# NVIDIAGameWorks/RayTracingDenoiser

Measured on AMD Instinct MI355X. Metric: Mpixels/s REBLUR_DIFFUSE_SPECULAR @1440p, higher is better.
Workload: dtype f32; 1 GPU; REBLUR_DIFFUSE_SPECULAR 2560x1440, default settings, analytic scene + 1rpp noise, moving camera; parallelism=1 GPU, storage=reference pool formats (fp16 history, R10G10B10A2 normals)

## Files before the change

raytracingdenoiser_amd/csrc/hip/kernels_reblur_ta.hip:

```cpp
#include "passes.h"
#include <climits>
#include <cstdio>
#include "reblur_device.h"

namespace nrdhip {

constexpr int TILE_X = 32;
constexpr int TILE_Y = 8;
static_assert(TILE_X == 32 && TILE_Y == 8, "planes.h LoadBlockTileBytes: a workgroup covers two 16x16 tiles of one tile row");
constexpr int BORDER = 1;
constexpr int BUF_X = TILE_X + 2 * BORDER;
constexpr int BUF_Y = TILE_Y + 2 * BORDER;
constexpr int BUF_STRIDE = BUF_X + 1;

#ifndef NRD_TA_WIN_H
#define NRD_TA_WIN_W 64
#define NRD_TA_WIN_H 16
#endif
#ifndef NRD_TA_SKY_FLAG_STORE
#define NRD_TA_SKY_FLAG_STORE 1
#endif
constexpr int WIN_W = NRD_TA_WIN_W;
constexpr int WIN_H = NRD_TA_WIN_H;

// ... 12 lines not shown
template <typename T>
NRD_D void WindowHistoryTexels(const HistoryFilter&, const uint2*, int, int, int, T&) {}
NRD_D void WindowFastTexels(const HistoryFilter& h, const uint32_t* win, int wx0, int wy0, const Plane& dims, int shift, BilinearTexelsR16F& t) {
    const int x0 = ClampI(h.ox, 0, dims.w - 1) - wx0, x1 = ClampI(h.ox + 1, 0, dims.w - 1) - wx0;
    const int y0 = (ClampI(h.oy, 0, dims.h - 1) - wy0) * WIN_W, y1 = (ClampI(h.oy + 1, 0, dims.h - 1) - wy0) * WIN_W;
    const uint32_t f00 = InBounds(dims, h.ox, h.oy) ? (win[y0 + x0] >> shift) & 0xFFFFu : 0u, f10 = InBounds(dims, h.ox + 1, h.oy) ? (win[y0 + x1] >> shift) & 0xFFFFu : 0u;
    const uint32_t f01 = InBounds(dims, h.ox, h.oy + 1) ? (win[y1 + x0] >> shift) & 0xFFFFu : 0u, f11 = InBounds(dims, h.ox + 1, h.oy + 1) ? (win[y1 + x1] >> shift) & 0xFFFFu : 0u;
    t.r0 = f00 | (f10 << 16);
    t.r1 = f01 | (f11 << 16);
    t.loaded = true;
}
template <typename T>
NRD_D void WindowFastTexels(const HistoryFilter&, const uint32_t*, int, int, const Plane&, int, T&) {}


template <bool DIFF, bool SPEC, bool PERF, int KIND, bool SH, int MODE>
__device__ __forceinline__ void ReblurTemporalAccumulationTile(const ReblurCB& cArg, TaPlanes P, const RowRange& rr, const int tileX, const int blockY) {
    typedef ReblurSignal<KIND> Sig;
    constexpr bool OCC = KIND == SIGNAL_OCCLUSION;
    typedef typename Sig::type S;
    __shared__ float4 s_Normal_Roughness[BUF_Y * BUF_STRIDE];
    __shared__ ReblurCB s_Constants;

    {
        const Plane size = P.viewZ, rgba16 = DIFF ? P.historyDiff : P.historySpec, r16 = DIFF ? P.historyDiffFast : P.historySpecFast;
        ShareSize(P.decodedNR, size), ShareSize(P.mv, size), ShareSize(P.prevViewZ, size), ShareSize(P.prevNormalRoughness, size), ShareSize(P.prevInternalData, size);
        ShareSize(P.inDiff, size), ShareSize(P.inSpec, size), ShareSize(P.inSpecHitDistForTracking, size), ShareSize(P.outData1, size), ShareSize(P.outData2, size);
        if (OCC) {
            const Plane sig = DIFF ? P.outDiff : P.outSpec;
            ShareSize(P.historyDiff, size), ShareSize(P.historySpec, size), ShareLayout(P.outDiff, sig), ShareLayout(P.outSpec, sig);
        } else {
            ShareLayout(P.historyDiff, rgba16), ShareLayout(P.historySpec, rgba16), ShareLayout(P.outDiff, rgba16), ShareLayout(P.outSpec, rgba16);
        }
        ShareLayout(P.historyDiffFast, r16), ShareLayout(P.historySpecFast, r16), ShareLayout(P.prevSpecHitDistForTracking, r16), ShareLayout(P.outDiffFast, r16), ShareLayout(P.outSpecFast, r16),
            ShareLayout(P.outSpecHitDistForTracking, r16);
    }
    __shared__ float s_HitDistForTracking[BUF_Y * BUF_STRIDE];
    constexpr int WIN_TEXELS = MODE == 1 ? WIN_W * WIN_H : 1;
    __shared__ float s_WinZ[WIN_TEXELS];
    __shared__ NrRaw s_WinN[WIN_TEXELS];
    __shared__ uint32_t s_WinId[WIN_TEXELS];
    __shared__ uint32_t s_WinFast[WIN_TEXELS];
    __shared__ uint2 s_WinDiff[WIN_TEXELS], s_WinSpec[WIN_TEXELS];
    __shared__ int s_WinBox[4][4];

    const int tx = threadIdx.x % TILE_X, ty = threadIdx.x / TILE_X;
    uint8_t* const tileFlag = (MODE == 1 && tileX < P.tileFlags.w && blockY < P.tileFlags.h) ? P.tileFlags.ptr + (uint32_t)blockY * P.tileFlags.pitch + (uint32_t)tileX : nullptr;
    const int px = tileX * TILE_X + tx, py = blockY * TILE_Y + ty;
    const int rw = cArg.gRectSizeMinusOne.x, rh = cArg.gRectSizeMinusOne.y;

    float preViewZ = 0.0f, preMaterialID = 0.0f;
    float4 preMv = F4(0.0f), preNormalAndRoughness = F4(0.0f);
    const uint32_t tileBytes = LoadBlockTileBytes(P.tiles, tileX, blockY);
    const bool preSky = TileByteIsSky(tileBytes, tx >> 4);
    {
        if (!TileBytesHaveGeometry<2>(tileBytes)) {
            if (NRD_TA_SKY_FLAG_STORE && MODE == 1 && threadIdx.x == 0 && tileFlag)
                *tileFlag = 0;
            return;
        }

        if (MODE == 1) {
            const int qx = min(px, rw), qy = min(max(py, 0), rh);
            preViewZ = LoadR32F(P.viewZ, qx, qy);
            preMv = LoadRGBA16F(P.mv, qx, qy);
            preNormalAndRoughness = LoadDecodedNormalRoughness(P.decodedNR, qx, qy, preMaterialID);
        }
        const int baseX = tileX * TILE_X - BORDER, baseY = blockY * TILE_Y - BORDER;
        for (int i = threadIdx.x; i < BUF_X * BUF_Y; i += TILE_X * TILE_Y) {
            int lx = i % BUF_X, ly = i / BUF_X;
            int gx = ClampI(baseX + lx, 0, rw), gy = ClampI(baseY + ly, 0, rh);
            float unusedMaterialID, texelViewZ;
            s_Normal_Roughness[ly * BUF_STRIDE + lx] = LoadDecodedNormalRoughness(P.decodedNR, gx, gy, unusedMaterialID, texelViewZ);
            if (SPEC) {
                const int shift = (OCC && cArg.gSpecCheckerboard != 2) ? 1 : 0;
                float hitDist = (OCC || cArg.gSpecPrepassBlurRadius == 0.0f) ? ExtractHitDist(Sig::Load(P.inSpec, gx >> shift, gy)) : LoadR16F(P.inSpecHitDistForTracking, gx, gy);
                if (shift) {
                    const int sx = min((gx & ~1) | (int)((cArg.gSpecCheckerboard ^ (uint32_t)gy ^ cArg.gFrameIndex) & 1u), rw);
                    LoadDecodedNormalRoughness(P.decodedNR, sx, gy, unusedMaterialID, texelViewZ);
                }
                if ((OCC || cArg.gSpecPrepassBlurRadius == 0.0f) && texelViewZ > cArg.gDenoisingRange)
                    hitDist = 0.0f;
                s_HitDistForTracking[ly * BUF_STRIDE + lx] = hitDist == 0.0f ? NRD_INF : hitDist;
            }
        }
        const uint32_t __attribute__((address_space(4)))* kernarg = (const uint32_t __attribute__((address_space(4)))*)__builtin_amdgcn_kernarg_segment_ptr();
        if (threadIdx.x < sizeof(ReblurCB) / 4)
            ((uint32_t*)&s_Constants)[threadIdx.x] = kernarg[threadIdx.x];
    }
    __syncthreads();
    const ReblurCB& c = s_Constants;
#define NRD_CONSTANTS_PHASE() asm volatile("" ::: "memory")

    const int lpx = MODE == 1 ? min(px, rw) : px, lpy = MODE == 1 ? min(py, rh) : py;
    bool active = !(px > rw || py > rh || py < rr.rowBegin || py >= rr.rowEnd);
    if (MODE != 1 && !active)
        return;
    if (MODE != 1) {
        if (preSky)
            return;
        preViewZ = LoadR32F(P.viewZ, lpx, lpy);
    }
    active = active && !preSky;
    const float viewZ = UnpackViewZ(c, preViewZ);
    active = active && !(viewZ > c.gDenoisingRange);
    if (MODE != 1 && !active)
        return;

    const float2 rectSize = ToF2(c.gRectSize), rectSizeInv = ToF2(c.gRectSizeInv), rectSizePrev = ToF2(c.gRectSizePrev);
    const float3 cameraDelta = ToF3(c.gCameraDelta);
    const float4 frustum = ToF4(c.gFrustum), frustumPrev = ToF4(c.gFrustumPrev), hitDistParams = ToF4(c.gHitDistParams);

    float2 pixelUv = F2(float(px) + 0.5f, float(py) + 0.5f) * rectSizeInv;
    float3 Xv = ReconstructViewPosition(pixelUv, frustum, viewZ, NRD_ORTHO_MODE(c));
    float3 X = RotateVector(c.gViewToWorld, Xv);

    float3 Navg = F3(0.0f);
    float hitDistForTracking = NRD_INF, roughnessM1 = 0.0f, roughnessM2 = 0.0f;
#pragma unroll
    for (int j = 0; j <= 2; j++) {
#pragma unroll
        for (int i = 0; i <= 2; i++) {
            int o = (ty + j) * BUF_STRIDE + tx + i;
            float4 nr = s_Normal_Roughness[o];
            if (i < 2 && j < 2)
                Navg = Navg + Xyz(nr);
            if (SPEC) {
                hitDistForTracking = Min(hitDistForTracking, s_HitDistForTracking[o]);
                float roughnessSq = nr.w * nr.w;
                roughnessM1 += roughnessSq;
                roughnessM2 += roughnessSq * roughnessSq;
            }
        }
    }
    Navg = Navg * 0.25f;

    if (MODE != 1)
        preNormalAndRoughness = LoadDecodedNormalRoughness(P.decodedNR, lpx, lpy, preMaterialID);
    float materialID = preMaterialID;
    float4 normalAndRoughness = preNormalAndRoughness;
    float3 N = Xyz(normalAndRoughness);
    float roughness = normalAndRoughness.w;

    float roughnessModified = 0.0f, roughnessSigma = 0.0f, hitDistNormalization = 0.0f;
    RngHash rng;
    if (SPEC) {
        roughnessModified = GetModifiedRoughnessFromNormalVariance(roughness, Navg);
        roughnessM1 = roughnessM1 * (1.0f / 9.0f);
        roughnessM2 = roughnessM2 * (1.0f / 9.0f);
        roughnessSigma = Sqrt(Abs(roughnessM2 - roughnessM1 * roughnessM1));

        rng.Initialize((uint32_t)px, (uint32_t)py, c.gFrameIndex);

        hitDistForTracking = hitDistForTracking == NRD_INF ? 0.0f : hitDistForTracking;
        hitDistNormalization = GetHitDistanceNormalization(viewZ, hitDistParams, roughness);
        hitDistForTracking *= (OCC || c.gSpecPrepassBlurRadius == 0.0f) ? hitDistNormalization : 1.0f;
        if (active)
            StoreR16F(P.outSpecHitDistForTracking, px, py, hitDistForTracking);
    }

    NRD_CONSTANTS_PHASE();
    float4 mvRaw = MODE == 1 ? preMv : LoadRGBA16F(P.mv, lpx, lpy);
    float3 mv = F3(mvRaw.x, mvRaw.y, mvRaw.z) * F3(c.gMvScale.x, c.gMvScale.y, c.gMvScale.z);
    float3 Xprev = X;
    float2 smbPixelUv = pixelUv + F2(mv.x, mv.y);
    if (c.gMvScale.w == 0.0f) {
        if (c.gMvScale.z == 0.0f)
            mv.z = AffineTransform(c.gWorldToViewPrev, X).z - viewZ;
        float viewZprev = viewZ + mv.z;
        float3 Xvprevlocal = ReconstructViewPosition(smbPixelUv, frustumPrev, viewZprev, NRD_ORTHO_MODE(c));
        Xprev = RotateVectorInverse(c.gWorldToViewPrev, Xvprevlocal) + cameraDelta;
    } else {
        Xprev = Xprev + mv;
        smbPixelUv = GetScreenUv(c.gWorldToClipPrev, Xprev);
    }

    TrackHistoryReach(P.historyReach, active ? HistoryReachRows(smbPixelUv.y, rectSizePrev.y, py) : 0.0f);

    float2 catromOrigin = GetCatmullRomOrigin(smbPixelUv, rectSizePrev);
    const int cx = (int)catromOrigin.x, cy = (int)catromOrigin.y;
    Bilinear smbBilinearFilter = GetBilinearFilter(smbPixelUv, rectSizePrev);
    const int bx = (int)smbBilinearFilter.origin.x, by = (int)smbBilinearFilter.origin.y;
    const float2 smbSamplePos = Sat(smbPixelUv) * rectSizePrev;
    HistoryFilter smbFilter = MakeHistoryGeometry(smbSamplePos, DIFF ? P.historyDiff : P.historySpec);
    typename Sig::HistoryTexels smbDiffTexels, smbSpecTexels;
    typename Sig::FastTexels smbDiffFastTexels, smbSpecFastTexels;
    S diff = Sig::Zero(), spec = Sig::Zero();
    float4 smbViewZ0, smbViewZ1, smbViewZ2, smbViewZ3;
    uint32_t id0[4], id1[4], id2[4], id3[4];
    NrRaw n00, n10, n01, n11;
    int wx0 = 0, wy0 = 0;
    if (MODE == 1) {
        const int W1 = P.prevViewZ.w - 1, H1 = P.prevViewZ.h - 1;
        int loX = INT_MAX, loY = INT_MAX, hiX = INT_MIN, hiY = INT_MIN;
        if (active) {
            loX = min(min(ClampI(cx, 0, W1), ClampI(bx, 0, W1)), min(smbFilter.x[0], ClampI(smbFilter.ox, 0, W1)));
            hiX = max(max(ClampI(cx + 3, 0, W1), ClampI(bx + 1, 0, W1)), max(smbFilter.x[3], ClampI(smbFilter.ox + 1, 0, W1)));
            loY = min(min(ClampI(cy, 0, H1), ClampI(by, 0, H1)), min(smbFilter.y[0], ClampI(smbFilter.oy, 0, H1)));
            hiY = max(max(ClampI(cy + 3, 0, H1), ClampI(by + 1, 0, H1)), max(smbFilter.y[3], ClampI(smbFilter.oy + 1, 0, H1)));
        }
#pragma unroll
        for (int m = 32; m >= 1; m >>= 1) {
            loX = min(loX, __shfl_xor(loX, m)), loY = min(loY, __shfl_xor(loY, m));
            hiX = max(hiX, __shfl_xor(hiX, m)), hiY = max(hiY, __shfl_xor(hiY, m));
        }
        const int lane = threadIdx.x & 63, wave = threadIdx.x >> 6;
        if (lane == 0)
            s_WinBox[wave][0] = loX, s_WinBox[wave][1] = loY, s_WinBox[wave][2] = hiX, s_WinBox[wave][3] = hiY;
        __syncthreads();
        loX = min(min(s_WinBox[0][0], s_WinBox[1][0]), min(s_WinBox[2][0], s_WinBox[3][0]));
        loY = min(min(s_WinBox[0][1], s_WinBox[1][1]), min(s_WinBox[2][1], s_WinBox[3][1]));
        hiX = max(max(s_WinBox[0][2], s_WinBox[1][2]), max(s_WinBox[2][2], s_WinBox[3][2]));
        hiY = max(max(s_WinBox[0][3], s_WinBox[1][3]), max(s_WinBox[2][3], s_WinBox[3][3]));
        const bool empty = hiX < loX;
        const int bw = hiX - loX + 1, bh = hiY - loY + 1;
        if (empty || bw > P.winMaxW || bh > P.winMaxH) {
            if (threadIdx.x == 0 && tileFlag)
                *tileFlag = empty ? 0 : 1;
            return;
        }
        if (threadIdx.x == 0 && tileFlag)
            *tileFlag = 0;
        wx0 = loX, wy0 = loY;
        if (lane < bw)
            for (int r = wave; r < bh; r += 4) {
                const int x = wx0 + lane, y = wy0 + r, o = r * WIN_W + lane;
                s_WinZ[o] = LoadR32F(P.prevViewZ, x, y);
                s_WinN[o] = LoadNrRaw(P.prevNormalRoughness, x, y);
                s_WinId[o] = LoadR16U(P.prevInternalData, x, y);
                s_WinFast[o] = (DIFF ? LoadR16U(P.historyDiffFast, x, y) : 0u) | (SPEC ? LoadR16U(P.historySpecFast, x, y) << 16 : 0u);
                if (DIFF)
                    s_WinDiff[o] = *TexelPtr<const uint2>(P.historyDiff, x, y);
                if (SPEC)
                    s_WinSpec[o] = *TexelPtr<const uint2>(P.historySpec, x, y);
            }
        __syncthreads();
        if (!active)
            return;
        int xo[4], yo[4];
#pragma unroll
        for (int i = 0; i < 4; i++)
            xo[i] = ClampI(cx + i, 0, W1) - wx0, yo[i] = (ClampI(cy + i, 0, H1) - wy0) * WIN_W;
#define WIN_Z(i, j) s_WinZ[yo[j] + xo[i]]
#define WIN_ID(i, j) s_WinId[yo[j] + xo[i]]
        smbViewZ0 = F4(WIN_Z(0, 0), WIN_Z(1, 0), WIN_Z(0, 1), WIN_Z(1, 1)), smbViewZ1 = F4(WIN_Z(2, 0), WIN_Z(3, 0), WIN_Z(2, 1), WIN_Z(3, 1));
        smbViewZ2 = F4(WIN_Z(0, 2), WIN_Z(1, 2), WIN_Z(0, 3), WIN_Z(1, 3)), smbViewZ3 = F4(WIN_Z(2, 2), WIN_Z(3, 2), WIN_Z(2, 3), WIN_Z(3, 3));
        id0[0] = WIN_ID(0, 0), id0[1] = WIN_ID(1, 0), id0[2] = WIN_ID(0, 1), id0[3] = WIN_ID(1, 1);
        id1[0] = WIN_ID(2, 0), id1[1] = WIN_ID(3, 0), id1[2] = WIN_ID(2, 1), id1[3] = WIN_ID(3, 1);
        id2[0] = WIN_ID(0, 2), id2[1] = WIN_ID(1, 2), id2[2] = WIN_ID(0, 3), id2[3] = WIN_ID(1, 3);
        id3[0] = WIN_ID(2, 2), id3[1] = WIN_ID(3, 2), id3[2] = WIN_ID(2, 3), id3[3] = WIN_ID(3, 3);
#undef WIN_Z
#undef WIN_ID
        const int nx0 = ClampI(bx, 0, W1) - wx0, nx1 = ClampI(bx + 1, 0, W1) - wx0, ny0 = (ClampI(by, 0, H1) - wy0) * WIN_W, ny1 = (ClampI(by + 1, 0, H1) - wy0) * WIN_W;
        n00 = InBounds(P.prevNormalRoughness, bx, by) ? s_WinN[ny0 + nx0] : NrRawZero();
        n10 = InBounds(P.prevNormalRoughness, bx + 1, by) ? s_WinN[ny0 + nx1] : NrRawZero();
        n01 = InBounds(P.prevNormalRoughness, bx, by + 1) ? s_WinN[ny1 + nx0] : NrRawZero();
        n11 = InBounds(P.prevNormalRoughness, bx + 1, by + 1) ? s_WinN[ny1 + nx1] : NrRawZero();
    } else {
        const bool footprintInterior = FootprintIsInterior(P.prevViewZ, cx, cy, 4, 4);
        const int fx4 = max(0, min(cx, P.prevViewZ.w - 4));
        const int fy0 = ClampI(cy, 0, P.prevViewZ.h - 1), fy1 = ClampI(cy + 1, 0, P.prevViewZ.h - 1), fy2 = ClampI(cy + 2, 0, P.prevViewZ.h - 1), fy3 = ClampI(cy + 3, 0, P.prevViewZ.h - 1);
        const float4 zr0 = LoadRowR32Fx4(P.prevViewZ, fx4, fy0), zr1 = LoadRowR32Fx4(P.prevViewZ, fx4, fy1), zr2 = LoadRowR32Fx4(P.prevViewZ, fx4, fy2), zr3 = LoadRowR32Fx4(P.prevViewZ, fx4, fy3);
        const uint2 ir0 = LoadRowR16x4Raw(P.prevInternalData, fx4, fy0), ir1 = LoadRowR16x4Raw(P.prevInternalData, fx4, fy1), ir2 = LoadRowR16x4Raw(P.prevInternalData, fx4, fy2), ir3 = LoadRowR16x4Raw(P.prevInternalData, fx4, fy3);
        const bool normalsInterior = FootprintIsInterior(P.prevNormalRoughness, bx, by, 2, 2);
        {
            const int nx = max(0, min(bx, P.prevNormalRoughness.w - 2));
            LoadRowNrRawx2(P.prevNormalRoughness, nx, ClampI(by, 0, P.prevNormalRoughness.h - 1), n00, n10);
            LoadRowNrRawx2(P.prevNormalRoughness, nx, ClampI(by + 1, 0, P.prevNormalRoughness.h - 1), n01, n11);
        }
        if (DIFF) {
            Sig::PrefetchHistory(smbFilter, P.historyDiff, smbDiffTexels, !PERF && KIND != SIGNAL_DIRECTIONAL_OCCLUSION);
            Sig::PrefetchFast(smbFilter, P.historyDiffFast, smbDiffFastTexels);
// ... 138 lines not shown
    int cbX0 = 0, cbX1 = 0;
    float2 wc = F2(0.0f, 0.0f);
    if (OCC && (c.gDiffCheckerboard != 2 || c.gSpecCheckerboard != 2)) {
        const int x0 = px > 0 ? px - 1 : 0, x1 = px < c.gRectSizeMinusOne.x ? px + 1 : c.gRectSizeMinusOne.x;
        const float viewZ0 = UnpackViewZ(c, LoadR32F(P.viewZ, x0, py)), viewZ1 = UnpackViewZ(c, LoadR32F(P.viewZ, x1, py));
        const float thr = GetDisocclusionThreshold(NRD_DISOCCLUSION_THRESHOLD, frustumSize, NoV);
        wc = F2(thr >= Abs(viewZ0 - viewZ) ? 1.0f : 0.0f, thr >= Abs(viewZ1 - viewZ) ? 1.0f : 0.0f);
        wc.x = (viewZ0 > c.gDenoisingRange || px < 1) ? 0.0f : wc.x;
        wc.y = (viewZ1 > c.gDenoisingRange || px >= c.gRectSizeMinusOne.x) ? 0.0f : wc.y;
        wc = wc * PositiveRcp(wc.x + wc.y);
        cbX0 = x0 >> 1;
        cbX1 = x1 >> 1;
    }

    if (DIFF) {
        if (MODE == 1)
            diff = Sig::Load(P.inDiff, px, py);
        float diffHistoryConfidence = smbFootprintQuality;
        if (c.gHasHistoryConfidence)
            diffHistoryConfidence *= LoadR8Unorm(P.diffConfidence, px, py);
        diffAccumSpeed *= Lerp(diffHistoryConfidence, 1.0f, Rcp(1.0f + diffAccumSpeed));
        diffAccumSpeed = Min(diffAccumSpeed, c.gMaxAccumulatedFrameNum);

        if (OCC && !diffHasData) {
            S d0 = Select(wc.x == 0.0f, Sig::Zero(), Sig::Load(P.inDiff, cbX0, py));
            S d1 = Select(wc.y == 0.0f, Sig::Zero(), Sig::Load(P.inDiff, cbX1, py));
            diff = d0 * wc.x + d1 * wc.y;
        }

        if (MODE == 1) {
            WindowHistoryTexels(smbFilter, s_WinDiff, wx0, wy0, WIN_W, smbDiffTexels);
            WindowFastTexels(smbFilter, s_WinFast, wx0, wy0, P.historyDiffFast, 0, smbDiffFastTexels);
        }
        S smbDiffHistory = Sig::FetchHistory(smbFilter, P.historyDiff, smbDiffTexels);
        float smbDiffFastHistory = Sig::FetchFastBilinear(smbFilter, P.historyDiffFast, smbDiffFastTexels);
        smbDiffHistory = ClampNegativeToZero(smbDiffHistory);

        float diffNonLinearAccumSpeed = Rcp(1.0f + diffAccumSpeed);
        if (!diffHasData)
            diffNonLinearAccumSpeed *= Lerp(1.0f - c.gCheckerboardResolveAccumSpeed, 1.0f, diffNonLinearAccumSpeed);
        S diffResult = MixHistoryAndCurrent(c, smbDiffHistory, diff, diffNonLinearAccumSpeed);
        float4 diffShResult = F4(0.0f);
        if (SH) {
            float4 smbDiffShHistory = FetchHistoryBilinearRGBA16F(smbFilter, P.historyDiffSh);
            diffShResult = MixHistoryAndCurrent(c, smbDiffShHistory, LoadRGBA16F(P.inDiffSh, px, py), diffNonLinearAccumSpeed);
        }

// ... 22 lines not shown
            diffFastNonLinearAccumSpeed *= Lerp(1.0f - c.gCheckerboardResolveAccumSpeed, 1.0f, diffFastNonLinearAccumSpeed);
        float diffFastResult = Lerp(smbDiffFastHistory, GetLuma(diff), diffFastNonLinearAccumSpeed);
        if (KIND == SIGNAL_RADIANCE) {
            float diffFastClamped = Min(diffFastResult, GetLuma(smbDiffHistory) * diffMaxRelativeIntensity * REBLUR_FIREFLY_SUPPRESSOR_FAST_RELATIVE_INTENSITY);
            diffFastResult = Lerp(diffFastResult, diffFastClamped, diffAntifireflyFactor);
        }
        Sig::StoreFast(P.outDiffFast, px, py, diffFastResult);
    }


    float specAccumSpeed = 0.0f, curvature = 0.0f, virtualHistoryAmount = 0.0f;
    if (SPEC) {
        S smbSpecHistory = Sig::Zero();
        float smbSpecFastHistory = 0.0f;
        float4 smbSpecShHistory = F4(0.0f);
        if (MODE == 1) {
            spec = Sig::Load(P.inSpec, px, py);
            WindowHistoryTexels(smbFilter, s_WinSpec, wx0, wy0, WIN_W, smbSpecTexels);
            WindowFastTexels(smbFilter, s_WinFast, wx0, wy0, P.historySpecFast, 16, smbSpecFastTexels);
            smbSpecHistory = Sig::FetchHistory(smbFilter, P.historySpec, smbSpecTexels);
            smbSpecFastHistory = Sig::FetchFastBilinear(smbFilter, P.historySpecFast, smbSpecFastTexels);
            if (SH)
                smbSpecShHistory = FetchHistoryBilinearRGBA16F(smbFilter, P.historySpecSh);
        }
        float specHistoryConfidence = smbFootprintQuality;
        if (c.gHasHistoryConfidence)
            specHistoryConfidence *= LoadR8Unorm(P.specConfidence, px, py);
        smbSpecAccumSpeed *= Lerp(specHistoryConfidence, 1.0f, Rcp(1.0f + smbSpecAccumSpeed));
        smbSpecAccumSpeed = Min(smbSpecAccumSpeed, c.gMaxAccumulatedFrameNum);

        if (OCC && !specHasData) {
            S s0 = Select(wc.x == 0.0f, Sig::Zero(), Sig::Load(P.inSpec, cbX0, py));
            S s1 = Select(wc.y == 0.0f, Sig::Zero(), Sig::Load(P.inSpec, cbX1, py));
            spec = s0 * wc.x + s1 * wc.y;
// ... 98 lines not shown
        vmbDelta = Div(vmbDelta, rectSizePrev);
        const float2 vmbPixelUvPrevTap = vmbPixelUv + vmbDelta * 1.0f * stepBetweenTaps;
        if (STOCHASTIC_NORMALS) {
            const int2 st1 = stochasticTexel(vmbPixelUvPrevTap);
            stochasticRaw1 = LoadNrRaw(P.prevNormalRoughness, st1.x, st1.y);
        } else
            vmbLinear1 = SampleLinearPrevNormalRoughness(P.prevNormalRoughness, vmbPixelUvPrevTap * resolutionScalePrev * prevNormalRoughnessSize);
        const LinearTaps hitDistTaps = MakeLinearTaps(vmbPixelUv * resolutionScalePrev * F2(float(P.prevSpecHitDistForTracking.w), float(P.prevSpecHitDistForTracking.h)));
        const bool hitDistInterior = FootprintIsInterior(P.prevSpecHitDistForTracking, hitDistTaps.x0, hitDistTaps.y0, 2, 2);
        const int hx = max(0, min(hitDistTaps.x0, P.prevSpecHitDistForTracking.w - 2));
        const uint32_t hdr0 = LoadRowR16x2Raw(P.prevSpecHitDistForTracking, hx, ClampI(hitDistTaps.y0, 0, P.prevSpecHitDistForTracking.h - 1));
        const uint32_t hdr1 = LoadRowR16x2Raw(P.prevSpecHitDistForTracking, hx, ClampI(hitDistTaps.y0 + 1, 0, P.prevSpecHitDistForTracking.h - 1));
        HistoryFilter vmbFilter = MakeHistoryGeometry(Sat(vmbPixelUv) * rectSizePrev, P.historySpec);
        typename Sig::HistoryTexels vmbSpecTexels;
        typename Sig::FastTexels vmbSpecFastTexels;
        if (MODE != 1) {
            Sig::PrefetchHistory(vmbFilter, P.historySpec, vmbSpecTexels, !PERF && KIND != SIGNAL_DIRECTIONAL_OCCLUSION);
            Sig::PrefetchFast(vmbFilter, P.historySpecFast, vmbSpecFastTexels);
        }

        float vz00 = vzr0.x, vz10 = vzr0.y, vz01 = vzr1.x, vz11 = vzr1.y;
        uint32_t vmbId00 = vidr0 & 0xFFFFu, vmbId10 = vidr0 >> 16, vmbId01 = vidr1 & 0xFFFFu, vmbId11 = vidr1 >> 16;
        uint32_t hd00 = hdr0 & 0xFFFFu, hd10 = hdr0 >> 16, hd01 = hdr1 & 0xFFFFu, hd11 = hdr1 >> 16;
        if (!vmbInterior) {
            const int x0 = ClampI(vx, 0, P.prevViewZ.w - 1), x1 = ClampI(vx + 1, 0, P.prevViewZ.w - 1), y0 = ClampI(vy, 0, P.prevViewZ.h - 1), y1 = ClampI(vy + 1, 0, P.prevViewZ.h - 1);
            vq00 = LoadNrRaw(P.prevNormalRoughness, x0, y0), vq10 = LoadNrRaw(P.prevNormalRoughness, x1, y0), vq01 = LoadNrRaw(P.prevNormalRoughness, x0, y1), vq11 = LoadNrRaw(P.prevNormalRoughness, x1, y1);
            vz00 = LoadR32F(P.prevViewZ, x0, y0), vz10 = LoadR32F(P.prevViewZ, x1, y0), vz01 = LoadR32F(P.prevViewZ, x0, y1), vz11 = LoadR32F(P.prevViewZ, x1, y1);
            vmbId00 = LoadR16U(P.prevInternalData, x0, y0), vmbId10 = LoadR16U(P.prevInternalData, x1, y0), vmbId01 = LoadR16U(P.prevInternalData, x0, y1), vmbId11 = LoadR16U(P.prevInternalData, x1, y1);
        }
        if (!hitDistInterior) {
            hd00 = FetchClampedR16U(P.prevSpecHitDistForTracking, hitDistTaps.x0, hitDistTaps.y0), hd10 = FetchClampedR16U(P.prevSpecHitDistForTracking, hitDistTaps.x0 + 1, hitDistTaps.y0);
// ... 112 lines not shown
            w.y = ComputeNonExponentialWeightWithSigma(vmbNormalAndRoughnessPrev.w * vmbNormalAndRoughnessPrev.w, relaxedRoughnessWeightParams.x, relaxedRoughnessWeightParams.y, roughnessSigma);
            if (STOCHASTIC_NORMALS)
                w = Lerp(F2(1.0f, 1.0f), w, Sat(stepBetweenTaps));
            w = Select(IsInScreenNearest(vmbPixelUvPrev) != 0.0f, w, F2(1.0f, 1.0f));

            virtualHistoryNormalBasedConfidence = Min(virtualHistoryNormalBasedConfidence, w.x);
            virtualHistoryRoughnessBasedConfidence = Min(virtualHistoryRoughnessBasedConfidence, w.y);
        }

        float virtualHistoryConfidenceForSmbRelaxation = virtualHistoryNormalBasedConfidence * virtualHistoryRoughnessBasedConfidence;
        float virtualHistoryConfidence = virtualHistoryNormalBasedConfidence * virtualHistoryRoughnessBasedConfidence * virtualHistoryParallaxBasedConfidence;
        virtualHistoryAmount *= virtualHistoryRoughnessBasedConfidence;
        TrackHistoryReach(P.historyReach, virtualHistoryAmount != 0.0f ? Max(HistoryReachRows(vmbPixelUv.y, rectSizePrev.y, py), HistoryReachRows(vmbPixelUvPrevTap.y, rectSizePrev.y, py)) : 0.0f);

        NRD_CONSTANTS_PHASE();
        if (MODE != 1) {
            smbSpecHistory = Sig::FetchHistory(smbFilter, P.historySpec, smbSpecTexels);
            smbSpecFastHistory = Sig::FetchFastBilinear(smbFilter, P.historySpecFast, smbSpecFastTexels);
        }

        float surfaceHistoryConfidence;
        {
            float a = Atan(Div(smbParallaxInPixelsMax * pixelSize, Length(X)));
            float nonLinearAccumSpeed = Rcp(1.0f + smbSpecAccumSpeed);
            float h = Lerp(ExtractHitDist(smbSpecHistory), ExtractHitDist(spec), nonLinearAccumSpeed) * hitDistNormalization;

            float tana0 = GetSpecularLobeTanHalfAngle(roughnessModified, NRD_MAX_PERCENT_OF_LOBE_VOLUME);
            tana0 *= Lerp(NoV, 1.0f, roughnessModified);
            tana0 *= nonLinearAccumSpeed;
            tana0 = Div(tana0, GetHitDistFactor(h, frustumSize) + NRD_EPS);

// ... 22 lines not shown
        float smbSpecAccumSpeedBoosted = Min(smbSpecAccumSpeed, smbBoostedMaxFrameNum);

        float vmbMaxFrameNum = c.gMaxAccumulatedFrameNum;
        vmbMaxFrameNum *= virtualHistoryConfidence;
        vmbMaxFrameNum = Min(vmbMaxFrameNum, maxResponsiveFrameNum.y);

        smbSpecAccumSpeed = Min(smbSpecAccumSpeed, smbMaxFrameNum);
        vmbSpecAccumSpeed = Min(vmbSpecAccumSpeed, vmbMaxFrameNum);

        float magic = vmbSpecAccumSpeed > smbSpecAccumSpeed ? 8.0f : 0.5f;
        virtualHistoryAmount *= 1.0f + Div(vmbSpecAccumSpeed - smbSpecAccumSpeed, magic * Max(vmbSpecAccumSpeed, smbSpecAccumSpeed) + 1.0f);
        virtualHistoryAmount = Sat(virtualHistoryAmount);

        NRD_CONSTANTS_PHASE();
        SetHistoryWeights(vmbFilter, vmbOcclusionWeights, vmbAllowCatRom);
        if (MODE == 1) {
            Sig::PrefetchHistory(vmbFilter, P.historySpec, vmbSpecTexels, !PERF && KIND != SIGNAL_DIRECTIONAL_OCCLUSION);
            Sig::PrefetchFast(vmbFilter, P.historySpecFast, vmbSpecFastTexels);
        }
        S vmbSpecHistory = Sig::FetchHistory(vmbFilter, P.historySpec, vmbSpecTexels);
        float vmbSpecFastHistory = Sig::FetchFastBilinear(vmbFilter, P.historySpecFast, vmbSpecFastTexels);

        smbSpecHistory = ClampNegativeToZero(smbSpecHistory);
        vmbSpecHistory = ClampNegativeToZero(vmbSpecHistory);

        float smbSpecNonLinearAccumSpeed = Rcp(1.0f + smbSpecAccumSpeed);
        float vmbSpecNonLinearAccumSpeed = Rcp(1.0f + vmbSpecAccumSpeed);
        if (!specHasData) {
            smbSpecNonLinearAccumSpeed *= Lerp(1.0f - c.gCheckerboardResolveAccumSpeed, 1.0f, smbSpecNonLinearAccumSpeed);
            vmbSpecNonLinearAccumSpeed *= Lerp(1.0f - c.gCheckerboardResolveAccumSpeed, 1.0f, vmbSpecNonLinearAccumSpeed);
        }

        S smbSpec = MixHistoryAndCurrent(c, smbSpecHistory, spec, smbSpecNonLinearAccumSpeed, roughnessModified);
        S vmbSpec = MixHistoryAndCurrent(c, vmbSpecHistory, spec, vmbSpecNonLinearAccumSpeed, roughnessModified);
        S specResult = Lerp(smbSpec, vmbSpec, virtualHistoryAmount);

        float4 specShResult = F4(0.0f);
        if (SH) {
            if (MODE != 1)
                smbSpecShHistory = FetchHistoryBilinearRGBA16F(smbFilter, P.historySpecSh);
            float4 vmbSpecShHistory = FetchHistoryBilinearRGBA16F(vmbFilter, P.historySpecSh);
            float4 specSh = LoadRGBA16F(P.inSpecSh, px, py);
            float4 smbShSpec = Lerp(smbSpecShHistory, specSh, smbSpecNonLinearAccumSpeed);
            float4 vmbShSpec = Lerp(vmbSpecShHistory, specSh, vmbSpecNonLinearAccumSpeed);
            specShResult = Lerp(smbShSpec, vmbShSpec, virtualHistoryAmount);
            specShResult.w = roughnessModified;
        }

        specAccumSpeed = Lerp(smbSpecAccumSpeedBoosted, vmbSpecAccumSpeed, virtualHistoryAmount);
        S specHistory = Lerp(smbSpecHistory, vmbSpecHistory, virtualHistoryAmount);

        float specMaxRelativeIntensity = 0.0f, specAntifireflyFactor = 0.0f;
        if (KIND == SIGNAL_RADIANCE) {
            specMaxRelativeIntensity = c.gFireflySuppressorMinRelativeScale + Div(REBLUR_FIREFLY_SUPPRESSOR_MAX_RELATIVE_INTENSITY, specAccumSpeed + 1.0f);
// ... 25 lines not shown
            specFastResult = Lerp(specFastResult, specFastClamped, specAntifireflyFactor);
        }
        Sig::StoreFast(P.outSpecFast, px, py, specFastResult);
    }

    NRD_CONSTANTS_PHASE();
    if (!OCC) {
        uint32_t packed = PackData2(fbits, curvature, virtualHistoryAmount);
        if (SPEC)
            StoreR32U(P.outData2, px, py, packed);
        else
            StoreR8U(P.outData2, px, py, packed);
    }

    StoreData1<DIFF, SPEC>(P.outData1, px, py, diffAccumSpeed, specAccumSpeed);
}

constexpr int FALLBACK_TILES = TILE_FLAG_GROUP;
template <bool DIFF, bool SPEC, bool PERF, int KIND, bool SH, int WAVES, int MODE>
__global__ __launch_bounds__(TILE_X* TILE_Y, WAVES) void ReblurTemporalAccumulationKernel(ReblurCB cArg, TaPlanes P, RowRange rr) {
    const int blockY = BlockTileY(rr, true);
    if (MODE != 2) {
        ReblurTemporalAccumulationTile<DIFF, SPEC, PERF, KIND, SH, MODE>(cArg, P, rr, BlockTileX(rr), blockY);
        return;
    }
    const int firstTile = (int)blockIdx.x * FALLBACK_TILES;
    if (!AnyTileFlagUniform(P.tileFlags, firstTile, min(blockY, P.tileFlags.h - 1)) || blockY >= P.tileFlags.h)
        return;
    const int endTile = min(FALLBACK_TILES, P.tileFlags.w - firstTile);
#pragma nounroll
    for (int k = 0; k < endTile; k++) {
        if (!TileFlagUniform(P.tileFlags, firstTile + k, blockY))
            continue;
        __syncthreads();
        ReblurTemporalAccumulationTile<DIFF, SPEC, PERF, KIND, SH, MODE>(cArg, P, rr, firstTile + k, blockY);
    }
}

template <bool DIFF, bool SPEC, bool PERF, int KIND, bool SH>
static const char* LaunchTemporalAccumulation(const PassArgs& a) {
    constexpr bool OCC = KIND == SIGNAL_OCCLUSION;
    const ReblurCB& c = *(const ReblurCB*)a.constants;
    if (c.gRectOrigin.x != 0 || c.gRectOrigin.y != 0)
        return "internal error: a pass was handed a non-zero rectOrigin";
    if (c.gOrthoMode != 0.0f)
        return "REBLUR: orthographic projection is not supported (SURVEY.md section 8c)";

    TaPlanes P = {};
    P.historyReach = a.historyReachWord;
    uint32_t k = 0;
// ... 42 lines not shown
            ok = ok && SameSize(P.historyDiff, size) && SameSize(P.historySpec, size) && SameLayout(P.outDiff, sig) && SameLayout(P.outSpec, sig);
        } else {
            ok = ok && SameLayout(P.historyDiff, rgba16) && SameLayout(P.historySpec, rgba16) && SameLayout(P.outDiff, rgba16) && SameLayout(P.outSpec, rgba16);
        }
        ok = ok && SameLayout(P.historyDiffFast, r16) && SameLayout(P.historySpecFast, r16) && SameLayout(P.prevSpecHitDistForTracking, r16) && SameLayout(P.outDiffFast, r16) &&
             SameLayout(P.outSpecFast, r16) && SameLayout(P.outSpecHitDistForTracking, r16);
        if (!ok)
            return "REBLUR temporal accumulation: planes of one frame must share their size (and pool planes of one format their pitch)";
    }

    RowGrid g = GridForRows(c.gRectSizeMinusOne.x + 1, c.gRectSizeMinusOne.y + 1, TILE_X, TILE_Y, a.rowBegin, a.rowEnd);
    static const int wavesEnv = getenv("NRD_HIP_TA_WAVES") ? atoi(getenv("NRD_HIP_TA_WAVES")) : 0;
    static const bool windowEnv = !(getenv("NRD_HIP_TA_WINDOW") && atoi(getenv("NRD_HIP_TA_WINDOW")) == 0);
    constexpr bool HAS_WINDOW = DIFF && SPEC && !PERF && KIND == SIGNAL_RADIANCE;
    if (HAS_WINDOW && windowEnv && !wavesEnv) {
        if (!a.tileFlags.ptr || (uint32_t)a.tileFlags.w * TILE_X < (uint32_t)P.viewZ.w || (uint32_t)a.tileFlags.h * TILE_Y < (uint32_t)P.viewZ.h ||
            a.tileFlags.pitch % TILE_FLAG_GROUP != 0 || ((uintptr_t)a.tileFlags.ptr & 255u) != 0)
            return "REBLUR temporal accumulation: the executor's tile-flag scratch is missing or too small";
        P.tileFlags = a.tileFlags;
        P.tileFlags.w = min(a.tileFlags.w, (int)((c.gRectSizeMinusOne.x + 1) + TILE_X - 1) / TILE_X);
        if (a.windowRegion)
            a.windowRegion[0] = P.tileFlags.w, a.windowRegion[1] = g.firstBlockY, a.windowRegion[2] = g.firstBlockY + (int)g.grid.y;
        static const char* limitEnv = getenv("NRD_HIP_TA_WINDOW_LIMIT");
        int limW = WIN_W, limH = WIN_H;
        if (limitEnv && sscanf(limitEnv, "%dx%d", &limW, &limH) != 2)
            limW = WIN_W, limH = WIN_H;
        P.winMaxW = limW < WIN_W ? limW : WIN_W;
        P.winMaxH = limH < WIN_H ? limH : WIN_H;
        LaunchPass(a, (ReblurTemporalAccumulationKernel<DIFF, SPEC, PERF, KIND, SH, 3, HAS_WINDOW ? 1 : 0>), g.grid, dim3(TILE_X * TILE_Y), c, P, MakeRowRange(g));
        dim3 fallbackGrid = g.grid;
        fallbackGrid.x = (unsigned)((P.tileFlags.w + FALLBACK_TILES - 1) / FALLBACK_TILES);
        LaunchPass(a, (ReblurTemporalAccumulationKernel<DIFF, SPEC, PERF, KIND, SH, SPEC ? 2 : 3, HAS_WINDOW ? 2 : 0>), fallbackGrid, dim3(TILE_X * TILE_Y), c, P, MakeRowRange(g));
        return nullptr;
    }
    const int waves = wavesEnv ? wavesEnv : (SPEC ? 2 : 3);
    if (waves >= 3)
        LaunchPass(a, (ReblurTemporalAccumulationKernel<DIFF, SPEC, PERF, KIND, SH, 3, 0>), g.grid, dim3(TILE_X * TILE_Y), c, P, MakeRowRange(g));
    else
        LaunchPass(a, (ReblurTemporalAccumulationKernel<DIFF, SPEC, PERF, KIND, SH, 2, 0>), g.grid, dim3(TILE_X * TILE_Y), c, P, MakeRowRange(g));
    return nullptr;
}

const PassEntry* GetReblurTemporalAccumulationPasses(uint32_t& num) {
    static const PassEntry k[] = {
#define REBLUR_TA_FAMILY(NAME, D, S)                                                                                 \
    {"REBLUR_" NAME "_TemporalAccumulation.cs", LaunchTemporalAccumulation<D, S, false, false, false>},            \
    {"REBLUR_Perf_" NAME "_TemporalAccumulation.cs", LaunchTemporalAccumulation<D, S, true, false, false>},        \
// ... 16 lines not shown
```

Baseline: 5295 Mpixels/s.

## Fold window-fallback tiles into the window kernel instead of a second launch

New measurement: 5301 Mpixels/s (median of 6 runs). Within noise of the previous version (+0.1%).

```diff
diff --git a/raytracingdenoiser_amd/csrc/hip/kernels_reblur_ta.hip b/raytracingdenoiser_amd/csrc/hip/kernels_reblur_ta.hip
--- a/raytracingdenoiser_amd/csrc/hip/kernels_reblur_ta.hip
+++ b/raytracingdenoiser_amd/csrc/hip/kernels_reblur_ta.hip
@@ -50,11 +50,15 @@
 NRD_D void WindowFastTexels(const HistoryFilter&, const uint32_t*, int, int, const Plane&, int, T&) {}
 
 
-template <bool DIFF, bool SPEC, bool PERF, int KIND, bool SH, int MODE>
-__device__ __forceinline__ void ReblurTemporalAccumulationTile(const ReblurCB& cArg, TaPlanes P, const RowRange& rr, const int tileX, const int blockY) {
+
+template <bool DIFF, bool SPEC, bool PERF, int KIND, bool SH, int MODE, bool SLOW>
+__device__ __forceinline__ bool ReblurTemporalAccumulationTile(const ReblurCB& cArg, TaPlanes P, const RowRange& rr, const int tileX, const int blockY) {
     typedef ReblurSignal<KIND> Sig;
     constexpr bool OCC = KIND == SIGNAL_OCCLUSION;
     typedef typename Sig::type S;
+    static_assert(!SLOW || MODE == 1, "SLOW is the second body of the window kernel");
+    constexpr bool WINDOW = MODE == 1 && !SLOW;
+    constexpr bool LATE = MODE == 1;
     __shared__ float4 s_Normal_Roughness[BUF_Y * BUF_STRIDE];
     __shared__ ReblurCB s_Constants;
 
@@ -72,7 +76,7 @@
             ShareLayout(P.outSpecHitDistForTracking, r16);
     }
     __shared__ float s_HitDistForTracking[BUF_Y * BUF_STRIDE];
-    constexpr int WIN_TEXELS = MODE == 1 ? WIN_W * WIN_H : 1;
+    constexpr int WIN_TEXELS = WINDOW ? WIN_W * WIN_H : 1;
     __shared__ float s_WinZ[WIN_TEXELS];
     __shared__ NrRaw s_WinN[WIN_TEXELS];
     __shared__ uint32_t s_WinId[WIN_TEXELS];
@@ -81,7 +85,7 @@
     __shared__ int s_WinBox[4][4];
 
     const int tx = threadIdx.x % TILE_X, ty = threadIdx.x / TILE_X;
-    uint8_t* const tileFlag = (MODE == 1 && tileX < P.tileFlags.w && blockY < P.tileFlags.h) ? P.tileFlags.ptr + (uint32_t)blockY * P.tileFlags.pitch + (uint32_t)tileX : nullptr;
+    uint8_t* const tileFlag = (WINDOW && tileX < P.tileFlags.w && blockY < P.tileFlags.h) ? P.tileFlags.ptr + (uint32_t)blockY * P.tileFlags.pitch + (uint32_t)tileX : nullptr;
     const int px = tileX * TILE_X + tx, py = blockY * TILE_Y + ty;
     const int rw = cArg.gRectSizeMinusOne.x, rh = cArg.gRectSizeMinusOne.y;
 
@@ -91,12 +95,12 @@
     const bool preSky = TileByteIsSky(tileBytes, tx >> 4);
     {
         if (!TileBytesHaveGeometry<2>(tileBytes)) {
-            if (NRD_TA_SKY_FLAG_STORE && MODE == 1 && threadIdx.x == 0 && tileFlag)
+            if (NRD_TA_SKY_FLAG_STORE && WINDOW && threadIdx.x == 0 && tileFlag)
                 *tileFlag = 0;
-            return;
-        }
-
-        if (MODE == 1) {
+            return false;
+        }
+
+        if (WINDOW) {
             const int qx = min(px, rw), qy = min(max(py, 0), rh);
             preViewZ = LoadR32F(P.viewZ, qx, qy);
             preMv = LoadRGBA16F(P.mv, qx, qy);
@@ -127,21 +131,30 @@
     __syncthreads();
     const ReblurCB& c = s_Constants;
 #define NRD_CONSTANTS_PHASE() asm volatile("" ::: "memory")
-
-    const int lpx = MODE == 1 ? min(px, rw) : px, lpy = MODE == 1 ? min(py, rh) : py;
+#ifdef NRD_EMU
+#define NRD_TA_COMPUTE_HERE(x) ((void)0)
+#define NRD_TA_OPAQUE_SCALAR(x) ((void)0)
+#define NRD_TA_UNIFORM_FLAG(x) (x)
+#else
+#define NRD_TA_UNIFORM_FLAG(x) (__builtin_amdgcn_readfirstlane((int)(x)) != 0)
+#define NRD_TA_COMPUTE_HERE(x) asm volatile("" : "+v"(x))
+#define NRD_TA_OPAQUE_SCALAR(x) asm volatile("" : "+s"(x))
+#endif
+
+    const int lpx = WINDOW ? min(px, rw) : px, lpy = WINDOW ? min(py, rh) : py;
     bool active = !(px > rw || py > rh || py < rr.rowBegin || py >= rr.rowEnd);
-    if (MODE != 1 && !active)
-        return;
-    if (MODE != 1) {
+    if (!WINDOW && !active)
+        return false;
+    if (!WINDOW) {
         if (preSky)
-            return;
+            return false;
         preViewZ = LoadR32F(P.viewZ, lpx, lpy);
     }
     active = active && !preSky;
     const float viewZ = UnpackViewZ(c, preViewZ);
     active = active && !(viewZ > c.gDenoisingRange);
-    if (MODE != 1 && !active)
-        return;
+    if (!WINDOW && !active)
+        return false;
 
     const float2 rectSize = ToF2(c.gRectSize), rectSizeInv = ToF2(c.gRectSizeInv), rectSizePrev = ToF2(c.gRectSizePrev);
     const float3 cameraDelta = ToF3(c.gCameraDelta);
@@ -171,7 +184,7 @@
     }
     Navg = Navg * 0.25f;
 
-    if (MODE != 1)
+    if (!WINDOW)
         preNormalAndRoughness = LoadDecodedNormalRoughness(P.decodedNR, lpx, lpy, preMaterialID);
     float materialID = preMaterialID;
     float4 normalAndRoughness = preNormalAndRoughness;
@@ -185,6 +198,8 @@
         roughnessM1 = roughnessM1 * (1.0f / 9.0f);
         roughnessM2 = roughnessM2 * (1.0f / 9.0f);
         roughnessSigma = Sqrt(Abs(roughnessM2 - roughnessM1 * roughnessM1));
+        if (SLOW)
+            NRD_TA_COMPUTE_HERE(roughnessSigma);
 
         rng.Initialize((uint32_t)px, (uint32_t)py, c.gFrameIndex);
 
@@ -196,7 +211,7 @@
     }
 
     NRD_CONSTANTS_PHASE();
-    float4 mvRaw = MODE == 1 ? preMv : LoadRGBA16F(P.mv, lpx, lpy);
+    float4 mvRaw = WINDOW ? preMv : LoadRGBA16F(P.mv, lpx, lpy);
     float3 mv = F3(mvRaw.x, mvRaw.y, mvRaw.z) * F3(c.gMvScale.x, c.gMvScale.y, c.gMvScale.z);
     float3 Xprev = X;
     float2 smbPixelUv = pixelUv + F2(mv.x, mv.y);
@@ -226,8 +241,8 @@
     uint32_t id0[4], id1[4], id2[4], id3[4];
     NrRaw n00, n10, n01, n11;
     int wx0 = 0, wy0 = 0;
-    if (MODE == 1) {
-        const int W1 = P.prevViewZ.w - 1, H1 = P.prevViewZ.h - 1;
+    const int W1 = P.prevViewZ.w - 1, H1 = P.prevViewZ.h - 1;
+    if (WINDOW) {
         int loX = INT_MAX, loY = INT_MAX, hiX = INT_MIN, hiY = INT_MIN;
         if (active) {
             loX = min(min(ClampI(cx, 0, W1), ClampI(bx, 0, W1)), min(smbFilter.x[0], ClampI(smbFilter.ox, 0, W1)));
@@ -250,10 +265,10 @@
         hiY = max(max(s_WinBox[0][3], s_WinBox[1][3]), max(s_WinBox[2][3], s_WinBox[3][3]));
         const bool empty = hiX < loX;
         const int bw = hiX - loX + 1, bh = hiY - loY + 1;
-        if (empty || bw > P.winMaxW || bh > P.winMaxH) {
+        if (NRD_TA_UNIFORM_FLAG(empty || bw > P.winMaxW || bh > P.winMaxH)) {
             if (threadIdx.x == 0 && tileFlag)
                 *tileFlag = empty ? 0 : 1;
-            return;
+            return !empty;
         }
         if (threadIdx.x == 0 && tileFlag)
             *tileFlag = 0;
@@ -272,13 +287,16 @@
             }
         __syncthreads();
         if (!active)
-            return;
+            return false;
+    }
+    if (LATE) {
+        constexpr int ROW = WINDOW ? WIN_W : 1;
         int xo[4], yo[4];
 #pragma unroll
         for (int i = 0; i < 4; i++)
-            xo[i] = ClampI(cx + i, 0, W1) - wx0, yo[i] = (ClampI(cy + i, 0, H1) - wy0) * WIN_W;
-#define WIN_Z(i, j) s_WinZ[yo[j] + xo[i]]
-#define WIN_ID(i, j) s_WinId[yo[j] + xo[i]]
+            xo[i] = ClampI(cx + i, 0, W1) - wx0, yo[i] = (ClampI(cy + i, 0, H1) - wy0) * ROW;
+#define WIN_Z(i, j) (WINDOW ? s_WinZ[yo[j] + xo[i]] : LoadR32F(P.prevViewZ, xo[i], yo[j]))
+#define WIN_ID(i, j) (WINDOW ? s_WinId[yo[j] + xo[i]] : LoadR16U(P.prevInternalData, xo[i], yo[j]))
         smbViewZ0 = F4(WIN_Z(0, 0), WIN_Z(1, 0), WIN_Z(0, 1), WIN_Z(1, 1)), smbViewZ1 = F4(WIN_Z(2, 0), WIN_Z(3, 0), WIN_Z(2, 1), WIN_Z(3, 1));
         smbViewZ2 = F4(WIN_Z(0, 2), WIN_Z(1, 2), WIN_Z(0, 3), WIN_Z(1, 3)), smbViewZ3 = F4(WIN_Z(2, 2), WIN_Z(3, 2), WIN_Z(2, 3), WIN_Z(3, 3));
         id0[0] = WIN_ID(0, 0), id0[1] = WIN_ID(1, 0), id0[2] = WIN_ID(0, 1), id0[3] = WIN_ID(1, 1);
@@ -287,11 +305,13 @@
         id3[0] = WIN_ID(2, 2), id3[1] = WIN_ID(3, 2), id3[2] = WIN_ID(2, 3), id3[3] = WIN_ID(3, 3);
 #undef WIN_Z
 #undef WIN_ID
-        const int nx0 = ClampI(bx, 0, W1) - wx0, nx1 = ClampI(bx + 1, 0, W1) - wx0, ny0 = (ClampI(by, 0, H1) - wy0) * WIN_W, ny1 = (ClampI(by + 1, 0, H1) - wy0) * WIN_W;
-        n00 = InBounds(P.prevNormalRoughness, bx, by) ? s_WinN[ny0 + nx0] : NrRawZero();
-        n10 = InBounds(P.prevNormalRoughness, bx + 1, by) ? s_WinN[ny0 + nx1] : NrRawZero();
-        n01 = InBounds(P.prevNormalRoughness, bx, by + 1) ? s_WinN[ny1 + nx0] : NrRawZero();
-        n11 = InBounds(P.prevNormalRoughness, bx + 1, by + 1) ? s_WinN[ny1 + nx1] : NrRawZero();
+        const int nx0 = ClampI(bx, 0, W1) - wx0, nx1 = ClampI(bx + 1, 0, W1) - wx0, ny0 = (ClampI(by, 0, H1) - wy0) * ROW, ny1 = (ClampI(by + 1, 0, H1) - wy0) * ROW;
+#define WIN_N(x, y) (WINDOW ? s_WinN[y + x] : LoadNrRaw(P.prevNormalRoughness, x, y))
+        n00 = InBounds(P.prevNormalRoughness, bx, by) ? WIN_N(nx0, ny0) : NrRawZero();
+        n10 = InBounds(P.prevNormalRoughness, bx + 1, by) ? WIN_N(nx1, ny0) : NrRawZero();
+        n01 = InBounds(P.prevNormalRoughness, bx, by + 1) ? WIN_N(nx0, ny1) : NrRawZero();
+        n11 = InBounds(P.prevNormalRoughness, bx + 1, by + 1) ? WIN_N(nx1, ny1) : NrRawZero();
+#undef WIN_N
     } else {
         const bool footprintInterior = FootprintIsInterior(P.prevViewZ, cx, cy, 4, 4);
         const int fx4 = max(0, min(cx, P.prevViewZ.w - 4));
@@ -460,7 +480,7 @@
     }
 
     if (DIFF) {
-        if (MODE == 1)
+        if (LATE)
             diff = Sig::Load(P.inDiff, px, py);
         float diffHistoryConfidence = smbFootprintQuality;
         if (c.gHasHistoryConfidence)
@@ -474,9 +494,12 @@
             diff = d0 * wc.x + d1 * wc.y;
         }
 
-        if (MODE == 1) {
+        if (WINDOW) {
             WindowHistoryTexels(smbFilter, s_WinDiff, wx0, wy0, WIN_W, smbDiffTexels);
             WindowFastTexels(smbFilter, s_WinFast, wx0, wy0, P.historyDiffFast, 0, smbDiffFastTexels);
+        } else if (SLOW) {
+            Sig::PrefetchHistory(smbFilter, P.historyDiff, smbDiffTexels, !PERF && KIND != SIGNAL_DIRECTIONAL_OCCLUSION);
+            Sig::PrefetchFast(smbFilter, P.historyDiffFast, smbDiffFastTexels);
         }
         S smbDiffHistory = Sig::FetchHistory(smbFilter, P.historyDiff, smbDiffTexels);
         float smbDiffFastHistory = Sig::FetchFastBilinear(smbFilter, P.historyDiffFast, smbDiffFastTexels);
@@ -529,10 +552,15 @@
         S smbSpecHistory = Sig::Zero();
         float smbSpecFastHistory = 0.0f;
         float4 smbSpecShHistory = F4(0.0f);
-        if (MODE == 1) {
+        if (LATE) {
             spec = Sig::Load(P.inSpec, px, py);
-            WindowHistoryTexels(smbFilter, s_WinSpec, wx0, wy0, WIN_W, smbSpecTexels);
-            WindowFastTexels(smbFilter, s_WinFast, wx0, wy0, P.historySpecFast, 16, smbSpecFastTexels);
+            if (WINDOW) {
+                WindowHistoryTexels(smbFilter, s_WinSpec, wx0, wy0, WIN_W, smbSpecTexels);
+                WindowFastTexels(smbFilter, s_WinFast, wx0, wy0, P.historySpecFast, 16, smbSpecFastTexels);
+            } else {
+                Sig::PrefetchHistory(smbFilter, P.historySpec, smbSpecTexels, !PERF && KIND != SIGNAL_DIRECTIONAL_OCCLUSION);
+                Sig::PrefetchFast(smbFilter, P.historySpecFast, smbSpecFastTexels);
+            }
             smbSpecHistory = Sig::FetchHistory(smbFilter, P.historySpec, smbSpecTexels);
             smbSpecFastHistory = Sig::FetchFastBilinear(smbFilter, P.historySpecFast, smbSpecFastTexels);
             if (SH)
@@ -661,7 +689,7 @@
         HistoryFilter vmbFilter = MakeHistoryGeometry(Sat(vmbPixelUv) * rectSizePrev, P.historySpec);
         typename Sig::HistoryTexels vmbSpecTexels;
         typename Sig::FastTexels vmbSpecFastTexels;
-        if (MODE != 1) {
+        if (!LATE) {
             Sig::PrefetchHistory(vmbFilter, P.historySpec, vmbSpecTexels, !PERF && KIND != SIGNAL_DIRECTIONAL_OCCLUSION);
             Sig::PrefetchFast(vmbFilter, P.historySpecFast, vmbSpecFastTexels);
         }
@@ -804,7 +832,7 @@
         TrackHistoryReach(P.historyReach, virtualHistoryAmount != 0.0f ? Max(HistoryReachRows(vmbPixelUv.y, rectSizePrev.y, py), HistoryReachRows(vmbPixelUvPrevTap.y, rectSizePrev.y, py)) : 0.0f);
 
         NRD_CONSTANTS_PHASE();
-        if (MODE != 1) {
+        if (!LATE) {
             smbSpecHistory = Sig::FetchHistory(smbFilter, P.historySpec, smbSpecTexels);
             smbSpecFastHistory = Sig::FetchFastBilinear(smbFilter, P.historySpecFast, smbSpecFastTexels);
         }
@@ -857,7 +885,7 @@
 
         NRD_CONSTANTS_PHASE();
         SetHistoryWeights(vmbFilter, vmbOcclusionWeights, vmbAllowCatRom);
-        if (MODE == 1) {
+        if (LATE) {
             Sig::PrefetchHistory(vmbFilter, P.historySpec, vmbSpecTexels, !PERF && KIND != SIGNAL_DIRECTIONAL_OCCLUSION);
             Sig::PrefetchFast(vmbFilter, P.historySpecFast, vmbSpecFastTexels);
         }
@@ -880,7 +908,7 @@
 
         float4 specShResult = F4(0.0f);
         if (SH) {
-            if (MODE != 1)
+            if (!LATE)
                 smbSpecShHistory = FetchHistoryBilinearRGBA16F(smbFilter, P.historySpecSh);
             float4 vmbSpecShHistory = FetchHistoryBilinearRGBA16F(vmbFilter, P.historySpecSh);
             float4 specSh = LoadRGBA16F(P.inSpecSh, px, py);
@@ -936,26 +964,25 @@
     }
 
     StoreData1<DIFF, SPEC>(P.outData1, px, py, diffAccumSpeed, specAccumSpeed);
+    return false;
 }
 
-constexpr int FALLBACK_TILES = TILE_FLAG_GROUP;
 template <bool DIFF, bool SPEC, bool PERF, int KIND, bool SH, int WAVES, int MODE>
 __global__ __launch_bounds__(TILE_X* TILE_Y, WAVES) void ReblurTemporalAccumulationKernel(ReblurCB cArg, TaPlanes P, RowRange rr) {
-    const int blockY = BlockTileY(rr, true);
-    if (MODE != 2) {
-        ReblurTemporalAccumulationTile<DIFF, SPEC, PERF, KIND, SH, MODE>(cArg, P, rr, BlockTileX(rr), blockY);
-        return;
-    }
-    const int firstTile = (int)blockIdx.x * FALLBACK_TILES;
-    if (!AnyTileFlagUniform(P.tileFlags, firstTile, min(blockY, P.tileFlags.h - 1)) || blockY >= P.tileFlags.h)
-        return;
-    const int endTile = min(FALLBACK_TILES, P.tileFlags.w - firstTile);
-#pragma nounroll
-    for (int k = 0; k < endTile; k++) {
-        if (!TileFlagUniform(P.tileFlags, firstTile + k, blockY))
-            continue;
-        __syncthreads();
-        ReblurTemporalAccumulationTile<DIFF, SPEC, PERF, KIND, SH, MODE>(cArg, P, rr, firstTile + k, blockY);
+    const int tileX = BlockTileX(rr), blockY = BlockTileY(rr, true);
+    const bool declined = ReblurTemporalAccumulationTile<DIFF, SPEC, PERF, KIND, SH, MODE, false>(cArg, P, rr, tileX, blockY);
+    if constexpr (MODE == 1) {
+        if (!declined)
+            return;
+        struct KernArgs {
+            ReblurCB c;
+            TaPlanes P;
+            RowRange rr;
+        };
+        const KernArgs __attribute__((address_space(4)))* kernarg = (const KernArgs __attribute__((address_space(4)))*)__builtin_amdgcn_kernarg_segment_ptr();
+        NRD_TA_OPAQUE_SCALAR(kernarg);
+        const KernArgs* args = (const KernArgs*)kernarg;
+        ReblurTemporalAccumulationTile<DIFF, SPEC, PERF, KIND, SH, MODE, true>(args->c, args->P, args->rr, tileX, blockY);
     }
 }
 
@@ -1028,8 +1055,7 @@
     static const bool windowEnv = !(getenv("NRD_HIP_TA_WINDOW") && atoi(getenv("NRD_HIP_TA_WINDOW")) == 0);
     constexpr bool HAS_WINDOW = DIFF && SPEC && !PERF && KIND == SIGNAL_RADIANCE;
     if (HAS_WINDOW && windowEnv && !wavesEnv) {
-        if (!a.tileFlags.ptr || (uint32_t)a.tileFlags.w * TILE_X < (uint32_t)P.viewZ.w || (uint32_t)a.tileFlags.h * TILE_Y < (uint32_t)P.viewZ.h ||
-            a.tileFlags.pitch % TILE_FLAG_GROUP != 0 || ((uintptr_t)a.tileFlags.ptr & 255u) != 0)
+        if (!a.tileFlags.ptr || (uint32_t)a.tileFlags.w * TILE_X < (uint32_t)P.viewZ.w || (uint32_t)a.tileFlags.h * TILE_Y < (uint32_t)P.viewZ.h)
             return "REBLUR temporal accumulation: the executor's tile-flag scratch is missing or too small";
         P.tileFlags = a.tileFlags;
         P.tileFlags.w = min(a.tileFlags.w, (int)((c.gRectSizeMinusOne.x + 1) + TILE_X - 1) / TILE_X);
@@ -1042,9 +1068,6 @@
         P.winMaxW = limW < WIN_W ? limW : WIN_W;
         P.winMaxH = limH < WIN_H ? limH : WIN_H;
         LaunchPass(a, (ReblurTemporalAccumulationKernel<DIFF, SPEC, PERF, KIND, SH, 3, HAS_WINDOW ? 1 : 0>), g.grid, dim3(TILE_X * TILE_Y), c, P, MakeRowRange(g));
-        dim3 fallbackGrid = g.grid;
-        fallbackGrid.x = (unsigned)((P.tileFlags.w + FALLBACK_TILES - 1) / FALLBACK_TILES);
-        LaunchPass(a, (ReblurTemporalAccumulationKernel<DIFF, SPEC, PERF, KIND, SH, SPEC ? 2 : 3, HAS_WINDOW ? 2 : 0>), fallbackGrid, dim3(TILE_X * TILE_Y), c, P, MakeRowRange(g));
         return nullptr;
     }
     const int waves = wavesEnv ? wavesEnv : (SPEC ? 2 : 3);
```
